# CrashCartCapital/rust-local-rag

Hardware: AMD Instinct MI355X
Metric: queries/sec, 768-d cosine top-100 over 10M chunks (single query, f32) (higher is better)
Workload: dtype f32

## Files before the change

### rust-local-rag_amd/csrc/exact.hip

```cpp
#include "common.h"
#include "exact_dot.h"
#include "staged_dot.h"
#include "sort_emit.h"
#include "kernels.h"
#include "../../include/rlr_gpu.h"

#include <algorithm>
#include <atomic>
#include <cstdlib>
#include <cstring>

namespace rlr {

namespace {

__device__ inline void stage_query(float *s_q, const float *__restrict__ query, uint32_t dim)
{
    for (uint32_t i = threadIdx.x; i < dim; i += blockDim.x)
        s_q[i] = query[i];
    __syncthreads();
}

template <bool F16>
__global__ __launch_bounds__(64) void rescore_kernel(const float4 *__restrict__ rows, uint32_t pitch16,
                                                     uint32_t dim, const float *__restrict__ query,
                                                     const uint32_t *__restrict__ cand,
                                                     const SelectState *__restrict__ st,
                                                     uint64_t *__restrict__ packed_out, uint32_t n_pad)
{
    extern __shared__ __attribute__((aligned(16))) float s_q[];
    stage_query(s_q, query, dim);
    const uint32_t n = min(st->n_cand, st->cap);
    const uint32_t i = blockIdx.x * 64 + threadIdx.x;
    if (i >= n_pad)
        return;
    if (i >= n) {
        packed_out[i] = 0;
        return;
    }
    const uint32_t r = cand[i];
    const float s = dot_ref_row<F16>(rows + static_cast<size_t>(r) * pitch16, s_q, dim);
    packed_out[i] = pack_result(s, r);
}

template <bool F16>
__global__ __launch_bounds__(256) void rescore_staged_kernel(const float4 *__restrict__ rows, uint32_t pitch16,
                                                             uint32_t dim, const float *__restrict__ query,
                                                             const uint32_t *__restrict__ cand,
                                                             const SelectState *__restrict__ st,
                                                             uint64_t *__restrict__ packed_out, uint32_t cpb,
                                                             uint32_t *__restrict__ hist_clear)
{
    extern __shared__ __attribute__((aligned(16))) float s_mem[];
    const uint32_t q_floats = (dim + 7) & ~7u;
    float *s_q = s_mem;
    float *s_p = s_mem + q_floats;
    const uint32_t tid = threadIdx.x;
    const uint32_t gid = blockIdx.x * 256 + tid;
    if (hist_clear && gid < 2 * kHistBins)
        hist_clear[gid] = 0;
    const uint32_t n = min(st->n_cand, st->cap);
    const uint32_t base = blockIdx.x * cpb;
    if (base >= n)
        return;
    const uint32_t cnt = min(cpb, n - base);
    __shared__ uint32_t s_cand[16];
    for (uint32_t i = tid; i < q_floats; i += 256)
        s_q[i] = i < dim ? query[i] : 0.0f;
    if (tid < cnt)
        s_cand[tid] = cand[base + tid];
    __syncthreads();
    const float sc = staged_reference_dot<F16>(rows, pitch16, dim, s_q, s_p, s_cand, cnt, tid);
    if (tid < cnt)
        packed_out[base + tid] = pack_result(sc, s_cand[tid]);
}

template <bool F16>
__global__ __launch_bounds__(256) void batch_rescore_kernel(const float4 *__restrict__ rows, uint32_t pitch16,
                                                            uint32_t dim, const float *__restrict__ queries,
                                                            uint32_t q_pitch, uint64_t *__restrict__ band,
                                                            uint32_t band_stride, const SelectState *__restrict__ st,
                                                            uint32_t cpb)
{
    extern __shared__ __attribute__((aligned(16))) float s_mem[];
    const uint32_t q_floats = (dim + 7) & ~7u;
    float *s_q = s_mem;
    float *s_p = s_mem + q_floats;
    __shared__ uint32_t s_cand[16];
    const uint32_t tid = threadIdx.x;
    const uint32_t q = blockIdx.y;
    const uint32_t n = st[q].pad;
    if (blockIdx.x * cpb >= n)
        return;
    const float *query = queries + static_cast<size_t>(q) * q_pitch;
    for (uint32_t i = tid; i < q_floats; i += 256)
        s_q[i] = i < dim ? query[i] : 0.0f;
    uint64_t *b = band + static_cast<size_t>(q) * band_stride;
    for (uint32_t base = blockIdx.x * cpb; base < n; base += gridDim.x * cpb) {
        const uint32_t cnt = min(cpb, n - base);
        __syncthreads();
        if (tid < cnt)
            s_cand[tid] = 0xFFFFFFFFu - static_cast<uint32_t>(b[base + tid] & 0xFFFFFFFFu);
        __syncthreads();
        const float sc = staged_reference_dot<F16>(rows, pitch16, dim, s_q, s_p, s_cand, cnt, tid);
        if (tid < cnt)
            b[base + tid] = pack_result(sc, s_cand[tid]);
    }
}

template <bool F16>
__global__ __launch_bounds__(64) void score_rows_kernel(const float4 *__restrict__ rows, uint32_t pitch16,
                                                        uint32_t dim, const float *__restrict__ query,
                                                        const uint32_t *__restrict__ list, uint32_t n,
                                                        float *__restrict__ out, const uint32_t *__restrict__ n_dev,
                                                        uint32_t n_rows_clamp)
{
    extern __shared__ __attribute__((aligned(16))) float s_q[];
    stage_query(s_q, query, dim);
    if (n_dev)
        n = min(n, *n_dev);
    const uint32_t i = blockIdx.x * 64 + threadIdx.x;
    if (i >= n)
        return;
    const uint32_t r = list[i] < n_rows_clamp ? list[i] : 0u;
    out[i] = dot_ref_row<F16>(rows + static_cast<size_t>(r) * pitch16, s_q, dim);
}

template <bool F16>
__global__ __launch_bounds__(64) void score_rows_batch_kernel(const float4 *__restrict__ rows, uint32_t pitch16, uint32_t dim,
                                                              const float *__restrict__ queries, uint32_t q_pitch,
                                                              const uint32_t *__restrict__ list, uint32_t stride,
                                                              float *__restrict__ out, const uint32_t *__restrict__ n_dev,
                                                              uint32_t n_dev_stride, uint32_t n_rows_clamp)
{
    const uint32_t q = blockIdx.y;
    const uint32_t n = min(stride, n_dev[static_cast<size_t>(q) * n_dev_stride]);
    if (blockIdx.x * 64 >= n)
        return;
    extern __shared__ __attribute__((aligned(16))) float s_q[];
    stage_query(s_q, queries + static_cast<size_t>(q) * q_pitch, dim);
    const uint32_t i = blockIdx.x * 64 + threadIdx.x;
    if (i >= n)
        return;
    const size_t at = static_cast<size_t>(q) * stride + i;
    const uint32_t r = list[at] < n_rows_clamp ? list[at] : 0u;
    out[at] = dot_ref_row<F16>(rows + static_cast<size_t>(r) * pitch16, s_q, dim);
}

template <bool F16>
__global__ __launch_bounds__(256) void score_rows_staged_kernel(const float4 *__restrict__ rows, uint32_t pitch16, uint32_t dim,
                                                               const float *__restrict__ query,
                                                               const uint32_t *__restrict__ list, uint32_t n,
                                                               float *__restrict__ out, uint32_t cpb,
                                                               const uint32_t *__restrict__ n_dev, uint32_t n_rows_clamp)
{
    extern __shared__ __attribute__((aligned(16))) float s_mem[];
    const uint32_t q_floats = (dim + 7) & ~7u;
    float *s_q = s_mem;
    float *s_p = s_mem + q_floats;
    __shared__ uint32_t s_cand[16];
    const uint32_t tid = threadIdx.x;
    const uint32_t base = blockIdx.x * cpb;
    if (n_dev)
        n = min(n, *n_dev);
    if (base >= n)
        return;
    const uint32_t cnt = min(cpb, n - base);
    for (uint32_t i = tid; i < q_floats; i += 256)
        s_q[i] = i < dim ? query[i] : 0.0f;
    if (tid < cnt) {
        const uint32_t r = list[base + tid];
        s_cand[tid] = r < n_rows_clamp ? r : 0u;
    }
    __syncthreads();
    const float sc = staged_reference_dot<F16>(rows, pitch16, dim, s_q, s_p, s_cand, cnt, tid);
    if (tid < cnt)
        out[base + tid] = sc;
}

__global__ __launch_bounds__(64) void sumsq_kernel(const float *__restrict__ staging, uint32_t n,
                                                   uint32_t dim, float *__restrict__ sumsq)
{
    const uint32_t r = blockIdx.x * 64 + threadIdx.x;
    if (r >= n)
        return;
    const float *v = staging + static_cast<size_t>(r) * dim;
    float s = 0.0f;
    for (uint32_t c = 0; c < dim; ++c) {
        float p = v[c] * v[c];
        s = s + p;
    }
    sumsq[r] = s;
}

__device__ inline float sqrt_rn(float x)
{
    float y = __builtin_sqrtf(x);
    const double xd = static_cast<double>(x);
#pragma unroll
    for (int it = 0; it < 2; ++it) {
        const uint32_t yb = __builtin_bit_cast(uint32_t, y);
        const float up = __builtin_bit_cast(float, yb + 1u);
        const float dn = __builtin_bit_cast(float, yb - 1u);
        const double m_hi = 0.5 * (static_cast<double>(y) + static_cast<double>(up));
        const double m_lo = 0.5 * (static_cast<double>(y) + static_cast<double>(dn));
        if (xd > m_hi * m_hi)
            y = up;
        else if (xd < m_lo * m_lo)
            y = dn;
    }
    return y;
}

__device__ inline float ref_scale(float v, float norm_sq, int do_normalize)
{
    if (do_normalize && norm_sq > 1e-20f)
        return __fdiv_rn(v, sqrt_rn(norm_sq));
    return v;
}

template <bool F16>
__global__ __launch_bounds__(256) void scale_store_kernel(const float *__restrict__ staging,
                                                          const float *__restrict__ sumsq, uint32_t n,
                                                          uint32_t dim, int do_normalize,
                                                          void *__restrict__ rows_out, uint32_t pitch16)
{
    const uint32_t pitch_e = F16 ? pitch16 * 8 : pitch16 * 4;
    const size_t total = static_cast<size_t>(n) * pitch_e;
    const size_t stride = static_cast<size_t>(gridDim.x) * 256;
    for (size_t i = static_cast<size_t>(blockIdx.x) * 256 + threadIdx.x; i < total; i += stride) {
        const uint32_t r = static_cast<uint32_t>(i / pitch_e);
        const uint32_t c = static_cast<uint32_t>(i - static_cast<size_t>(r) * pitch_e);
        float v = 0.0f;
        if (c < dim)
            v = ref_scale(staging[static_cast<size_t>(r) * dim + c], do_normalize ? sumsq[r] : 0.0f,
                          do_normalize);
        if constexpr (F16)
            static_cast<_Float16 *>(rows_out)[i] = static_cast<_Float16>(v);
        else
            static_cast<float *>(rows_out)[i] = v;
    }
}

__device__ inline uint64_t mix64(uint64_t z)
{
    z = (z ^ (z >> 30)) * 0xBF58476D1CE4E5B9ULL;
    z = (z ^ (z >> 27)) * 0x94D049BB133111EBULL;
    return z ^ (z >> 31);
}

__device__ inline int32_t ih4(uint64_t h)
{
    return static_cast<int32_t>((h & 0xFFFF) + ((h >> 16) & 0xFFFF) + ((h >> 32) & 0xFFFF) + (h >> 48)) - 131070;
}

__device__ inline float synth_raw(uint64_t s, uint64_t row, uint32_t col, uint32_t d, uint32_t n_clusters)
{
    const uint64_t idx = row * static_cast<uint64_t>(d) + col;
    int32_t t = ih4(mix64(s + (idx + 1) * 0x9E3779B97F4A7C15ULL));
    const bool tight = (n_clusters & 0x80000000u) != 0;
    n_clusters &= 0x7FFFFFFFu;
    if (n_clusters) {
        const uint64_t cl = mix64(s ^ (row + 0x632BE59BD9B4E019ULL)) % n_clusters;
        const uint64_t cidx = cl * static_cast<uint64_t>(d) + col;
        const int32_t c = ih4(mix64((s ^ 0xC1A57E55C1A57E55ULL) + (cidx + 1) * 0x9E3779B97F4A7C15ULL));
        if (tight)
            t = t / 16;
        t += 2 * c;
    }
    return static_cast<float>(t) * (1.0f / 65536.0f);
}

__global__ __launch_bounds__(64) void synth_sumsq_kernel(uint64_t s, uint64_t row0, uint32_t n, uint32_t dim,
                                                         uint32_t n_clusters, float *__restrict__ sumsq)
{
    const uint32_t r = blockIdx.x * 64 + threadIdx.x;
    if (r >= n)
        return;
    float acc = 0.0f;
    for (uint32_t c = 0; c < dim; ++c) {
        const float v = synth_raw(s, row0 + r, c, dim, n_clusters);
        float p = v * v;
        acc = acc + p;
    }
    sumsq[r] = acc;
}

template <bool F16>
__global__ __launch_bounds__(256) void synth_store_kernel(uint64_t s, uint64_t row0, uint32_t n, uint32_t dim,
                                                          uint32_t n_clusters, const float *__restrict__ sumsq,
                                                          void *__restrict__ rows_out, uint32_t pitch16)
{
    const uint32_t pitch_e = F16 ? pitch16 * 8 : pitch16 * 4;
    const size_t total = static_cast<size_t>(n) * pitch_e;
    const size_t stride = static_cast<size_t>(gridDim.x) * 256;
    for (size_t i = static_cast<size_t>(blockIdx.x) * 256 + threadIdx.x; i < total; i += stride) {
        const uint32_t r = static_cast<uint32_t>(i / pitch_e);
        const uint32_t c = static_cast<uint32_t>(i - static_cast<size_t>(r) * pitch_e);
        float v = 0.0f;
        if (c < dim)
            v = ref_scale(synth_raw(s, row0 + r, c, dim, n_clusters), sumsq[r], 1);
        if constexpr (F16)
            static_cast<_Float16 *>(rows_out)[i] = static_cast<_Float16>(v);
        else
            static_cast<float *>(rows_out)[i] = v;
    }
}

template <bool F16>
__global__ __launch_bounds__(256) void gather_f32_kernel(const void *__restrict__ rows, uint32_t pitch16,
                                                         uint32_t dim, const uint32_t *__restrict__ list,
                                                         uint32_t n, float *__restrict__ out)
{
    const size_t total = static_cast<size_t>(n) * dim;
    const size_t stride = static_cast<size_t>(gridDim.x) * 256;
    for (size_t i = static_cast<size_t>(blockIdx.x) * 256 + threadIdx.x; i < total; i += stride) {
        const uint32_t k = static_cast<uint32_t>(i / dim);
        const uint32_t c = static_cast<uint32_t>(i - static_cast<size_t>(k) * dim);
        const size_t r = list[k];
        if constexpr (F16)
            out[i] = h2f(static_cast<const uint16_t *>(rows)[r * pitch16 * 8 + c]);
        else
            out[i] = static_cast<const float *>(rows)[r * pitch16 * 4 + c];
    }
}

__global__ __launch_bounds__(256) void compact_rows_kernel(const float4 *__restrict__ src, float4 *__restrict__ dst,
                                                           uint32_t pitch16, const uint32_t *__restrict__ keep,
                                                           uint32_t n_keep)
{
    const size_t total = static_cast<size_t>(n_keep) * pitch16;
    const size_t stride = static_cast<size_t>(gridDim.x) * 256;
    for (size_t i = static_cast<size_t>(blockIdx.x) * 256 + threadIdx.x; i < total; i += stride) {
        const uint32_t k = static_cast<uint32_t>(i / pitch16);
        const uint32_t u = static_cast<uint32_t>(i - static_cast<size_t>(k) * pitch16);
        dst[i] = src[static_cast<size_t>(keep[k]) * pitch16 + u];
    }
}

__device__ inline bool finite_f(float x)
{
    return (__builtin_bit_cast(uint32_t, x) & 0x7F800000u) != 0x7F800000u;
}

__device__ inline float gram_entry(float dot)
{
    return finite_f(dot) ? dot : -__builtin_inff();
}

template <int SRC>
__device__ inline float4 gram_load4(const float *pool, const void *rows, uint32_t pitch16, uint32_t dim, uint32_t row, uint32_t col)
{
    if constexpr (SRC == 2) {
        const uint2 h = *reinterpret_cast<const uint2 *>(static_cast<const uint16_t *>(rows) + static_cast<size_t>(row) * pitch16 * 8 + col);
        return make_float4(h2f(static_cast<uint16_t>(h.x)), h2f(static_cast<uint16_t>(h.x >> 16)), h2f(static_cast<uint16_t>(h.y)),
                           h2f(static_cast<uint16_t>(h.y >> 16)));
    } else if constexpr (SRC == 1) {
        return *reinterpret_cast<const float4 *>(static_cast<const float *>(rows) + static_cast<size_t>(row) * pitch16 * 4 + col);
    } else {
        return *reinterpret_cast<const float4 *>(pool + static_cast<size_t>(row) * dim + col);
    }
}


template <int R, int SRC, int GK>
__global__ __launch_bounds__(256) void gram_tiled_kernel(const float *__restrict__ pool, uint32_t P, uint32_t dim,
                                                         float *__restrict__ gram, const void *__restrict__ rows,
                                                         uint32_t pitch16, const uint32_t *__restrict__ list)
{
    constexpr int kGT = 16 * R;
    constexpr int kGK = GK, kGPitch = GK + 4;
    __shared__ __attribute__((aligned(16))) float sa[kGT * kGPitch];
    __shared__ __attribute__((aligned(16))) float sb[kGT * kGPitch];
    if constexpr (SRC == 0)
        pool += static_cast<size_t>(blockIdx.z) * P * dim;
    else
        list += static_cast<size_t>(blockIdx.z) * P;
    gram += static_cast<size_t>(blockIdx.z) * P * P;
    uint32_t bi = 0, rem = blockIdx.x;
    while (rem > bi) {
        rem -= bi + 1;
        ++bi;
    }
    const uint32_t bj = rem;
    const uint32_t i0 = bi * kGT, j0 = bj * kGT;
    const uint32_t t = threadIdx.x, ty = t >> 4, tx = t & 15;
    float acc[R][R];
#pragma unroll
    for (int a = 0; a < R; ++a)
#pragma unroll
        for (int b = 0; b < R; ++b)
            acc[a][b] = 0.0f;
    const bool vec = (dim & 3u) == 0;
    constexpr int kPre = 2 * kGT * (kGK / 4) / 256;
    float4 pre[kPre];
    uint32_t src_row[kPre];
#pragma unroll
    for (int u = 0; u < kPre; ++u) {
        const uint32_t r = (t + 256 * u) / (kGK / 4);
        const uint32_t row = min(r >= kGT ? j0 + (r - kGT) : i0 + r, P - 1);
        src_row[u] = SRC == 0 ? row : list[row];
    }
    auto fetch = [&](uint32_t k0) {
        const uint32_t kc = min(static_cast<uint32_t>(kGK), dim - k0);
        if (vec) {
#pragma unroll
            for (int u = 0; u < kPre; ++u) {
                const uint32_t idx = t + 256 * u;
                const uint32_t r = idx / (kGK / 4), c4 = idx % (kGK / 4);
                const uint32_t row = r >= kGT ? j0 + (r - kGT) : i0 + r;
                const float4 v = gram_load4<SRC>(pool, rows, pitch16, dim, src_row[u], min(k0 + c4 * 4, dim - 4));
                pre[u] = (row < P && c4 * 4 < kc) ? v : make_float4(0.0f, 0.0f, 0.0f, 0.0f);
            }
            return;
        }
#pragma unroll
        for (int u = 0; u < kPre; ++u) {
            const uint32_t idx = t + 256 * u;
            const uint32_t r = idx / (kGK / 4), c4 = idx % (kGK / 4);
            const uint32_t row = r >= kGT ? j0 + (r - kGT) : i0 + r;
            float4 v = make_float4(0.0f, 0.0f, 0.0f, 0.0f);
            if (row < P && c4 * 4 < kc) {
                const uint32_t col = k0 + c4 * 4;
                if constexpr (SRC == 2) {
                    const uint16_t *src = static_cast<const uint16_t *>(rows) + static_cast<size_t>(src_row[u]) * pitch16 * 8 + col;
                    v.x = h2f(src[0]);
                    if (c4 * 4 + 1 < kc) v.y = h2f(src[1]);
                    if (c4 * 4 + 2 < kc) v.z = h2f(src[2]);
                    if (c4 * 4 + 3 < kc) v.w = h2f(src[3]);
                } else {
                    const float *src = SRC == 0 ? pool + static_cast<size_t>(row) * dim + col
                                                : static_cast<const float *>(rows) + static_cast<size_t>(src_row[u]) * pitch16 * 4 + col;
                    v.x = src[0];
                    if (c4 * 4 + 1 < kc) v.y = src[1];
                    if (c4 * 4 + 2 < kc) v.z = src[2];
                    if (c4 * 4 + 3 < kc) v.w = src[3];
                }
            }
            pre[u] = v;
        }
    };
    auto stash = [&]() {
#pragma unroll
        for (int u = 0; u < kPre; ++u) {
            const uint32_t idx = t + 256 * u;
            const uint32_t r = idx / (kGK / 4), c4 = idx % (kGK / 4);
            float *dst = (r >= kGT ? sb + (r - kGT) * kGPitch : sa + r * kGPitch) + c4 * 4;
            *reinterpret_cast<float4 *>(dst) = pre[u];
        }
    };
    fetch(0);
    stash();
    __syncthreads();
    for (uint32_t k0 = 0; k0 < dim; k0 += kGK) {
        const uint32_t kc = min(static_cast<uint32_t>(kGK), dim - k0);
        const bool more = k0 + kGK < dim;
        if (more)
            fetch(k0 + kGK);
        const uint32_t n4 = kc / 4;
        constexpr int kUnroll = R == 1 ? 8 : 1;
#pragma unroll kUnroll
        for (uint32_t c = 0; c < n4; ++c) {
            float4 xa[R], yb[R];
#pragma unroll
            for (int a = 0; a < R; ++a)
                xa[a] = reinterpret_cast<const float4 *>(sa + (ty + 16 * a) * kGPitch)[c];
#pragma unroll
            for (int b = 0; b < R; ++b)
                yb[b] = reinterpret_cast<const float4 *>(sb + (tx + 16 * b) * kGPitch)[c];
#pragma unroll
            for (int a = 0; a < R; ++a)
#pragma unroll
                for (int b = 0; b < R; ++b) {
                    float p;
                    p = xa[a].x * yb[b].x; acc[a][b] = acc[a][b] + p;
                    p = xa[a].y * yb[b].y; acc[a][b] = acc[a][b] + p;
                    p = xa[a].z * yb[b].z; acc[a][b] = acc[a][b] + p;
                    p = xa[a].w * yb[b].w; acc[a][b] = acc[a][b] + p;
                }
        }
        for (uint32_t e = n4 * 4; e < kc; ++e) {
#pragma unroll
            for (int a = 0; a < R; ++a)
#pragma unroll
                for (int b = 0; b < R; ++b) {
                    const float p = sa[(ty + 16 * a) * kGPitch + e] * sb[(tx + 16 * b) * kGPitch + e];
                    acc[a][b] = acc[a][b] + p;
                }
        }
        __syncthreads();
        if (more) {
            stash();
            __syncthreads();
        }
    }
#pragma unroll
    for (int a = 0; a < R; ++a)
#pragma unroll
        for (int b = 0; b < R; ++b) {
            const uint32_t ri = i0 + ty + 16 * a, cj = j0 + tx + 16 * b;
            if (ri < P && cj < P) {
                const float g = gram_entry(acc[a][b]);
                gram[static_cast<size_t>(ri) * P + cj] = g;
                gram[static_cast<size_t>(cj) * P + ri] = g;
            }
        }
}

__global__ __launch_bounds__(64) void mmr_greedy_kernel(const float *__restrict__ gram,
                                                        const float *__restrict__ scores, uint32_t P,
                                                        uint32_t k, float lambda, uint32_t *__restrict__ out_order,
                                                        float *__restrict__ out_mmr, uint32_t *__restrict__ out_n)
{
    extern __shared__ __attribute__((aligned(16))) unsigned char s_raw[];
    uint32_t *rem = reinterpret_cast<uint32_t *>(s_raw);
    float *max_sim = reinterpret_cast<float *>(s_raw) + P;
    float *rel = reinterpret_cast<float *>(s_raw) + 2 * P;
    const uint32_t lane = threadIdx.x;
    if (P == 0) {
        if (lane == 0)
            *out_n = 0;
        return;
    }
    for (uint32_t p = lane; p < P; p += 64) {
        rem[p] = p;
        max_sim[p] = 0.0f;
        rel[p] = scores[p];
    }
    __syncthreads();
    uint32_t n_rem = P, n_sel = 0;
    uint32_t last = rem[0];
    __syncthreads();
    if (lane == 0) {
        out_order[0] = last;
        out_mmr[0] = __builtin_bit_cast(float, 0x7FC00000u);
        rem[0] = rem[P - 1];
    }
    n_sel = 1;
    n_rem = P - 1;
    __syncthreads();

    const float one_minus = 1.0f - lambda;
    while (n_sel < k && n_rem > 0) {
        const float *g_last = gram + static_cast<size_t>(last) * P;
        uint64_t best = 0;
        for (uint32_t p = lane; p < n_rem; p += 64) {
            const uint32_t c = rem[p];
            const float sim = g_last[c];
            float ms = max_sim[c];
            if (finite_f(sim))
                ms = fmaxf(ms, sim);
            max_sim[c] = ms;
            const float r = rel[c];
            if (!finite_f(r))
                continue;
            const float t0 = one_minus * r;
            const float t1 = lambda * ms;
            float m = t0 - t1;
            if (!finite_f(m))
                continue;
            if (m == 0.0f)
                m = 0.0f;
            const uint64_t cand = (static_cast<uint64_t>(score_key(m)) << 32) | (0xFFFFFFFFu - p);
            if (cand > best)
                best = cand;
        }
#pragma unroll
        for (int off = 32; off > 0; off >>= 1) {
            const uint32_t hi = __shfl_xor(static_cast<uint32_t>(best >> 32), off);
            const uint32_t lo = __shfl_xor(static_cast<uint32_t>(best & 0xFFFFFFFFu), off);
            const uint64_t other = (static_cast<uint64_t>(hi) << 32) | lo;
            if (other > best)
                best = other;
        }
        if (best == 0)
            break;
        const uint32_t best_p = 0xFFFFFFFFu - static_cast<uint32_t>(best & 0xFFFFFFFFu);
        __syncthreads();
        last = rem[best_p];
        __syncthreads();
        if (lane == 0) {
            out_order[n_sel] = last;
            out_mmr[n_sel] = one_minus * rel[last] - lambda * max_sim[last];
            rem[best_p] = rem[n_rem - 1];
        }
        n_sel++;
        n_rem--;
        __syncthreads();
    }
    if (lane == 0)
        *out_n = n_sel;
}

template <typename Order>
__device__ __forceinline__ void emit_result_block(const MmrEmit &emit, uint32_t n_sel, uint32_t lane, Order order)
{
    const uint32_t status = emit.info[1];
    const uint32_t n = status ? 0u : min(n_sel, emit.k_cap);
    uint32_t chk = 0;
    for (uint32_t i = lane; i < n; i += 64) {
        const uint32_t o = order(i);
        const uint32_t w0 = emit.list[o], w1 = __builtin_bit_cast(uint32_t, emit.cosv[o]);
        const uint32_t w2 = __builtin_bit_cast(uint32_t, emit.comb[o]);
        const uint32_t w3 = emit.lexv ? __builtin_bit_cast(uint32_t, emit.lexv[o]) : 0u;
        emit.h_out[block_value(emit.k_cap, kBlockRow, i)] = w0;
        emit.h_out[block_value(emit.k_cap, kBlockCos, i)] = w1;
        emit.h_out[block_value(emit.k_cap, kBlockComb, i)] = w2;
        emit.h_out[block_value(emit.k_cap, kBlockLex, i)] = w3;
        chk += result_chk_term(w0, block_value(emit.k_cap, kBlockRow, i)) + result_chk_term(w1, block_value(emit.k_cap, kBlockCos, i)) +
               result_chk_term(w2, block_value(emit.k_cap, kBlockComb, i)) + result_chk_term(w3, block_value(emit.k_cap, kBlockLex, i));
    }
    __threadfence_system();
#pragma unroll
    for (int off = 32; off > 0; off >>= 1)
        chk += static_cast<uint32_t>(__shfl_xor(static_cast<int>(chk), off));
    if (lane == 0) {
        emit.h_out[block_n(emit.k_cap)] = n;
        emit.h_out[block_status(emit.k_cap)] = status;
        emit.h_out[block_chk(emit.k_cap)] = block_chk_tail(chk, n, status, emit.k_cap);
        __threadfence_system();
        emit.h_out[block_done(emit.k_cap)] = kBlockDone;
    }
}

__device__ __forceinline__ void emit_empty_block(const MmrEmit &emit)
{
    const uint32_t status = emit.info[1];
    emit.h_out[block_n(emit.k_cap)] = 0;
    emit.h_out[block_status(emit.k_cap)] = status;
    emit.h_out[block_chk(emit.k_cap)] = block_chk_tail(0u, 0u, status, emit.k_cap);
    __threadfence_system();
    emit.h_out[block_done(emit.k_cap)] = kBlockDone;
}

template <int J>
__device__ inline float lane_max_skip_nan(const float (&v)[J])
{
    float best = -__builtin_inff();
    int j = 0;
#pragma unroll
    for (; j + 1 < J; j += 2)
        asm("v_max3_f32 %0, %1, %2, %3" : "=v"(best) : "v"(best), "v"(v[j]), "v"(v[j + 1]));
    if (j < J)
        asm("v_max_f32 %0, %1, %2" : "=v"(best) : "v"(best), "v"(v[j]));
    return best;
}

template <int J>
__global__ __launch_bounds__(256) void mmr_greedy_lazy_kernel(const float *__restrict__ gram, const float *__restrict__ scores,
                                                              uint32_t P, uint32_t k, float lambda,
                                                              uint32_t *__restrict__ out_order, float *__restrict__ out_mmr,
                                                              uint32_t *__restrict__ out_n, const uint32_t *__restrict__ sizes,
                                                              MmrEmit emit)
{
    constexpr uint32_t kSlots = 64 * J;
    __shared__ uint2 s_log[kSlots];
    __shared__ uint16_t s_rem[kSlots], s_posof[kSlots];
    {
        const uint32_t stride = P;
        gram += static_cast<size_t>(blockIdx.x) * stride * stride;
        scores += static_cast<size_t>(blockIdx.x) * stride;
        out_order += static_cast<size_t>(blockIdx.x) * stride;
        out_mmr += static_cast<size_t>(blockIdx.x) * stride;
        out_n += blockIdx.x;
    }
    const uint32_t g_stride = P;
    if (sizes)
        P = sizes[blockIdx.x];
    if (P == 0) {
        if (threadIdx.x == 0) {
            *out_n = 0;
            if (emit.h_out)
                emit_empty_block(emit);
        }
        return;
    }
    {
        const float4 *g4 = reinterpret_cast<const float4 *>(gram);
        const uint32_t n4 = (P * g_stride) / 4;
        float warm = 0.0f;
        for (uint32_t i = threadIdx.x * 8; i < n4; i += 256 * 8)
            warm += g4[i].x;
        asm volatile("" ::"v"(warm));
    }
    __syncthreads();
    if (threadIdx.x >= 64)
        return;
    const uint32_t lane = threadIdx.x;
    for (uint32_t c = lane; c < P; c += 64) {
        s_rem[c] = static_cast<uint16_t>(c);
        s_posof[c] = static_cast<uint16_t>(c);
    }
    float t0[J], ms[J];
    uint32_t idx[J];
    const float one_minus = 1.0f - lambda;
    const float nan_f = __builtin_bit_cast(float, 0x7FC00000u);
    const float neg_inf = -__builtin_inff();
#pragma unroll
    for (int j = 0; j < J; ++j) {
        const uint32_t c = lane + 64 * j;
        idx[j] = min(c, P - 1);
        const float t = one_minus * scores[idx[j]];
        t0[j] = ((c < P) & (c != 0) & finite_f(t)) ? t : nan_f;
        ms[j] = 0.0f;
    }
    uint32_t n_sel = 1, last = 0, replayed = 0;
    s_log[0] = make_uint2(0u, 0x7FC00000u);
    while (n_sel < k && n_sel < P) {
        const float *g_last = gram + static_cast<size_t>(last) * g_stride;
        float sim[J];
#pragma unroll
        for (int j = 0; j < J; ++j)
            sim[j] = g_last[idx[j]];
        float m0[J];
#pragma unroll
        for (int j = 0; j < J; ++j) {
            ms[j] = sim[j] > ms[j] ? sim[j] : ms[j];
            const float t1 = lambda * ms[j];
            m0[j] = t0[j] - t1;
        }
        float wm = wave_max_f32_no_nan(lane_max_skip_nan<J>(m0));
        if (wm == __builtin_inff()) {
#pragma unroll
            for (int j = 0; j < J; ++j)
                m0[j] = finite_f(m0[j]) ? m0[j] : nan_f;
            wm = wave_max_f32_no_nan(lane_max_skip_nan<J>(m0));
        }
        if (wm == neg_inf)
            break;
        auto take = [&](const bool (&hit)[J]) {
            uint32_t win = 0;
#pragma unroll
            for (int j = 0; j < J; ++j) {
                win = hit[j] ? lane + 64 * j + 1 : win;
                t0[j] = hit[j] ? nan_f : t0[j];
            }
            const int src = __builtin_ctzll(__ballot(win != 0));
            last = static_cast<uint32_t>(__builtin_amdgcn_readlane(static_cast<int>(win), src)) - 1;
            float wm_raw = wm;
            if (wm == 0.0f) {
                float z = 0.0f;
#pragma unroll
                for (int j = 0; j < J; ++j)
                    z = hit[j] ? m0[j] : z;
                wm_raw = __builtin_bit_cast(float, __builtin_amdgcn_readlane(__builtin_bit_cast(int, z), src));
            }
            s_log[n_sel] = make_uint2(last, __builtin_bit_cast(uint32_t, wm_raw));
            __builtin_amdgcn_fence(__ATOMIC_RELEASE, "wavefront");
            __builtin_amdgcn_wave_barrier();
            n_sel++;
        };
        bool hit[J];
        uint32_t holders = 0;
#pragma unroll
        for (int j = 0; j < J; ++j) {
            hit[j] = m0[j] == wm;
            holders += static_cast<uint32_t>(__builtin_popcountll(__ballot(hit[j])));
        }
        if (holders == 1) {
            take(hit);
            continue;
        }
        if (lane == 0) {
            for (uint32_t i = replayed; i < n_sel; ++i) {
                const uint32_t w = s_log[i].x, n = P - i;
                const uint32_t p = s_posof[w], moved = s_rem[n - 1];
                s_rem[p] = static_cast<uint16_t>(moved);
                s_posof[moved] = static_cast<uint16_t>(p);
            }
        }
        __builtin_amdgcn_fence(__ATOMIC_RELEASE, "wavefront");
        __builtin_amdgcn_wave_barrier();
        __builtin_amdgcn_fence(__ATOMIC_ACQUIRE, "wavefront");
        replayed = n_sel;
        uint32_t pj[J], bp = 0xFFFFFFFFu;
#pragma unroll
        for (int j = 0; j < J; ++j) {
            pj[j] = hit[j] ? static_cast<uint32_t>(s_posof[idx[j]]) : 0xFFFFFFFFu;
            bp = min(bp, pj[j]);
        }
        const uint32_t wp = wave_min_u32(bp);
        bool first[J];
#pragma unroll
        for (int j = 0; j < J; ++j)
            first[j] = pj[j] == wp;
        take(first);
    }
    for (uint32_t i = lane; i < n_sel; i += 64) {
        const uint2 e = s_log[i];
        out_order[i] = e.x;
        out_mmr[i] = __builtin_bit_cast(float, e.y);
    }
    if (lane == 0)
        *out_n = n_sel;
    if (emit.h_out)
        emit_result_block(emit, n_sel, lane, [&](uint32_t i) { return s_log[i].x; });
}

uint32_t ew_blocks(size_t total)
{
    size_t b = (total + 255) / 256;
    if (b > 256 * 16) b = 256 * 16;
    return b ? static_cast<uint32_t>(b) : 1u;
}

}

hipError_t launch_rescore(const void *rows, uint32_t pitch16, uint32_t dim, int dtype, const float *query,
                          const uint32_t *cand, const SelectState *st, uint64_t *packed_out, uint32_t n_pad,
                          hipStream_t s)
{
    const uint32_t blocks = (n_pad + 63) / 64;
    const size_t lds = static_cast<size_t>(dim) * sizeof(float);
    const float4 *r4 = static_cast<const float4 *>(rows);
    if (dtype == RLR_F16)
        hipLaunchKernelGGL(rescore_kernel<true>, dim3(blocks), dim3(64), lds, s, r4, pitch16, dim, query, cand, st,
                           packed_out, n_pad);
    else
        hipLaunchKernelGGL(rescore_kernel<false>, dim3(blocks), dim3(64), lds, s, r4, pitch16, dim, query, cand, st,
                           packed_out, n_pad);
    return hipGetLastError();
}

bool launch_rescore_staged(const void *rows, uint32_t pitch16, uint32_t dim, int dtype, const float *query,
                           const uint32_t *cand, const SelectState *st, uint64_t *packed_out, uint32_t n_max,
                           uint32_t *hist_clear, hipStream_t s, hipError_t *err)
{
    const size_t q_bytes = static_cast<size_t>((dim + 7) & ~7u) * sizeof(float);
    const size_t row_bytes = q_bytes + 16;
    if (pitch16 * (dtype == RLR_F16 ? 8u : 4u) < ((dim + 7) & ~7u))
        return false;
    uint32_t cpb = 8;
    while (cpb > 1 && q_bytes + cpb * row_bytes > 60 * 1024)
        cpb >>= 1;
    if (q_bytes + cpb * row_bytes > 60 * 1024)
        return false;
    const uint32_t blocks = std::max<uint32_t>((n_max + cpb - 1) / cpb, (2 * kHistBins + 255) / 256);
    const size_t lds = q_bytes + cpb * row_bytes;
    const float4 *r4 = static_cast<const float4 *>(rows);
    if (dtype == RLR_F16)
        hipLaunchKernelGGL(rescore_staged_kernel<true>, dim3(blocks), dim3(256), lds, s, r4, pitch16, dim, query, cand,
                           st, packed_out, cpb, hist_clear);
    else
        hipLaunchKernelGGL(rescore_staged_kernel<false>, dim3(blocks), dim3(256), lds, s, r4, pitch16, dim, query, cand,
                           st, packed_out, cpb, hist_clear);
    *err = hipGetLastError();
    return true;
}

bool batch_rescore_fits(uint32_t pitch16, uint32_t dim, int dtype)
{
    const size_t q_bytes = static_cast<size_t>((dim + 7) & ~7u) * sizeof(float);
    if (pitch16 * (dtype == RLR_F16 ? 8u : 4u) < ((dim + 7) & ~7u))
        return false;
    return 2 * q_bytes + 16 <= 60 * 1024;
}

bool launch_batch_rescore(const void *rows, uint32_t pitch16, uint32_t dim, int dtype, const float *queries,
                          uint32_t q_pitch, uint32_t n_queries, uint64_t *band, uint32_t band_stride,
                          const SelectState *st, hipStream_t s, hipError_t *err)
{
    const size_t q_bytes = static_cast<size_t>((dim + 7) & ~7u) * sizeof(float);
    const size_t row_bytes = q_bytes + 16;
    if (pitch16 * (dtype == RLR_F16 ? 8u : 4u) < ((dim + 7) & ~7u))
        return false;
    uint32_t cpb = 8;
    while (cpb > 1 && q_bytes + cpb * row_bytes > 60 * 1024)
        cpb >>= 1;
    if (q_bytes + cpb * row_bytes > 60 * 1024)
        return false;
    const size_t lds = q_bytes + cpb * row_bytes;
    const float4 *r4 = static_cast<const float4 *>(rows);
    const dim3 grid(32, n_queries);
    if (dtype == RLR_F16)
        hipLaunchKernelGGL(batch_rescore_kernel<true>, grid, dim3(256), lds, s, r4, pitch16, dim, queries, q_pitch, band,
                           band_stride, st, cpb);
    else
        hipLaunchKernelGGL(batch_rescore_kernel<false>, grid, dim3(256), lds, s, r4, pitch16, dim, queries, q_pitch, band,
                           band_stride, st, cpb);
    *err = hipGetLastError();
    return true;
}

hipError_t launch_score_rows(const void *rows, uint32_t pitch16, uint32_t dim, int dtype, const float *query,
                             const uint32_t *list, uint32_t n, float *cos_out, hipStream_t s, const uint32_t *n_dev,
                             uint32_t n_rows_clamp)
{
    if (n == 0)
        return hipSuccess;
    const float4 *r4 = static_cast<const float4 *>(rows);
    const size_t q_bytes = static_cast<size_t>((dim + 7) & ~7u) * sizeof(float);
    const size_t row_bytes = q_bytes + 16;
    uint32_t cpb = 8;
    while (cpb > 1 && q_bytes + cpb * row_bytes > 60 * 1024)
        cpb >>= 1;
    const bool fits = q_bytes + cpb * row_bytes <= 60 * 1024 && pitch16 * (dtype == RLR_F16 ? 8u : 4u) >= ((dim + 7) & ~7u);
    if (fits && n > 64) {
        const uint32_t blocks = (n + cpb - 1) / cpb;
        const size_t lds = q_bytes + cpb * row_bytes;
        if (dtype == RLR_F16)
            hipLaunchKernelGGL(score_rows_staged_kernel<true>, dim3(blocks), dim3(256), lds, s, r4, pitch16, dim, query, list, n,
                               cos_out, cpb, n_dev, n_rows_clamp);
        else
            hipLaunchKernelGGL(score_rows_staged_kernel<false>, dim3(blocks), dim3(256), lds, s, r4, pitch16, dim, query, list, n,
                               cos_out, cpb, n_dev, n_rows_clamp);
        return hipGetLastError();
    }
    const uint32_t blocks = (n + 63) / 64;
    const size_t lds = static_cast<size_t>(dim) * sizeof(float);
    if (dtype == RLR_F16)
        hipLaunchKernelGGL(score_rows_kernel<true>, dim3(blocks), dim3(64), lds, s, r4, pitch16, dim, query, list, n,
                           cos_out, n_dev, n_rows_clamp);
    else
        hipLaunchKernelGGL(score_rows_kernel<false>, dim3(blocks), dim3(64), lds, s, r4, pitch16, dim, query, list, n,
                           cos_out, n_dev, n_rows_clamp);
    return hipGetLastError();
}

hipError_t launch_score_rows_batch(const void *rows, uint32_t pitch16, uint32_t dim, int dtype, const float *queries,
                                   uint32_t q_pitch, uint32_t n_queries, const uint32_t *list, uint32_t stride, float *cos_out,
                                   const uint32_t *n_dev, uint32_t n_dev_stride, uint32_t n_rows_clamp, hipStream_t s)
{
    if (stride == 0 || n_queries == 0)
        return hipSuccess;
    const float4 *r4 = static_cast<const float4 *>(rows);
    const dim3 grid((stride + 63) / 64, n_queries);
    const size_t lds = static_cast<size_t>(dim) * sizeof(float);
    if (dtype == RLR_F16)
        hipLaunchKernelGGL(score_rows_batch_kernel<true>, grid, dim3(64), lds, s, r4, pitch16, dim, queries, q_pitch, list, stride,
                           cos_out, n_dev, n_dev_stride, n_rows_clamp);
    else
        hipLaunchKernelGGL(score_rows_batch_kernel<false>, grid, dim3(64), lds, s, r4, pitch16, dim, queries, q_pitch, list, stride,
                           cos_out, n_dev, n_dev_stride, n_rows_clamp);
    return hipGetLastError();
}

hipError_t launch_normalize_store(float *staging, uint32_t n, uint32_t dim, int do_normalize, void *rows_out,
                                  uint32_t pitch16, int dtype, float *norm_tmp, hipStream_t s)
{
    if (n == 0)
        return hipSuccess;
    hipLaunchKernelGGL(sumsq_kernel, dim3((n + 63) / 64), dim3(64), 0, s, staging, n, dim, norm_tmp);
    const size_t total = static_cast<size_t>(n) * pitch16 * (dtype == RLR_F16 ? 8 : 4);
    if (dtype == RLR_F16)
        hipLaunchKernelGGL(scale_store_kernel<true>, dim3(ew_blocks(total)), dim3(256), 0, s, staging, norm_tmp, n,
                           dim, do_normalize, rows_out, pitch16);
    else
        hipLaunchKernelGGL(scale_store_kernel<false>, dim3(ew_blocks(total)), dim3(256), 0, s, staging, norm_tmp, n,
                           dim, do_normalize, rows_out, pitch16);
    return hipGetLastError();
}

hipError_t launch_synth(void *rows_out, uint32_t pitch16, uint32_t dim, int dtype, uint64_t row0, uint32_t n,
                        uint64_t seed, uint32_t n_clusters, float *norm_tmp, hipStream_t s)
{
    if (n == 0)
        return hipSuccess;
    uint64_t z = seed ^ 0x5EED5EED5EED5EEDULL;
    z = (z ^ (z >> 30)) * 0xBF58476D1CE4E5B9ULL;
    z = (z ^ (z >> 27)) * 0x94D049BB133111EBULL;
    z = z ^ (z >> 31);
    hipLaunchKernelGGL(synth_sumsq_kernel, dim3((n + 63) / 64), dim3(64), 0, s, z, row0, n, dim, n_clusters,
                       norm_tmp);
    const size_t total = static_cast<size_t>(n) * pitch16 * (dtype == RLR_F16 ? 8 : 4);
    if (dtype == RLR_F16)
        hipLaunchKernelGGL(synth_store_kernel<true>, dim3(ew_blocks(total)), dim3(256), 0, s, z, row0, n, dim,
                           n_clusters, norm_tmp, rows_out, pitch16);
    else
        hipLaunchKernelGGL(synth_store_kernel<false>, dim3(ew_blocks(total)), dim3(256), 0, s, z, row0, n, dim,
                           n_clusters, norm_tmp, rows_out, pitch16);
    return hipGetLastError();
}

hipError_t launch_gather_f32(const void *rows, uint32_t pitch16, uint32_t dim, int dtype, const uint32_t *list,
                             uint32_t n, float *out, hipStream_t s)
{
    if (n == 0)
        return hipSuccess;
    const size_t total = static_cast<size_t>(n) * dim;
    if (dtype == RLR_F16)
        hipLaunchKernelGGL(gather_f32_kernel<true>, dim3(ew_blocks(total)), dim3(256), 0, s, rows, pitch16, dim, list,
                           n, out);
    else
        hipLaunchKernelGGL(gather_f32_kernel<false>, dim3(ew_blocks(total)), dim3(256), 0, s, rows, pitch16, dim,
                           list, n, out);
    return hipGetLastError();
}

hipError_t launch_compact_rows(const void *src, void *dst, uint32_t pitch16, const uint32_t *keep, uint32_t n_keep,
                               hipStream_t s)
{
    if (n_keep == 0)
        return hipSuccess;
    const size_t total = static_cast<size_t>(n_keep) * pitch16;
    hipLaunchKernelGGL(compact_rows_kernel, dim3(ew_blocks(total)), dim3(256), 0, s,
                       static_cast<const float4 *>(src), static_cast<float4 *>(dst), pitch16, keep, n_keep);
    return hipGetLastError();
}

typedef float v32f __attribute__((ext_vector_type(32)));

__global__ __launch_bounds__(64) void gram_mfma_f32_kernel(const unsigned char *__restrict__ rows, uint32_t pitch_bytes,
                                                           uint32_t dim, const uint32_t *__restrict__ list, uint32_t P,
                                                           uint32_t n_pools, uint32_t jobs_per_pool, float *__restrict__ gram)
{
    constexpr int UPR = 4;
    constexpr int kGmPitch = UPR * 16 + 16;
    constexpr int kPer = 96 * UPR / 64;
    __shared__ __attribute__((aligned(16))) unsigned char s_rows[96 * kGmPitch];
    const uint32_t xcd = blockIdx.x & 7u, slot = blockIdx.x >> 3;
    const uint32_t pool = (slot / jobs_per_pool) * 8 + xcd;
    if (pool >= n_pools)
        return;
    const uint32_t nb = (P + 31) / 32;
    uint32_t p = 0, rem = slot % jobs_per_pool;
    while (rem >= nb - 2 * p) {
        rem -= nb - 2 * p;
        ++p;
    }
    const uint32_t I0 = 2 * p, J = 2 * p + rem;
    list += static_cast<size_t>(pool) * P;
    gram += static_cast<size_t>(pool) * P * P;
    const uint32_t lane = threadIdx.x;
    const unsigned char *src[kPer];
#pragma unroll
    for (int i = 0; i < kPer; ++i) {
        const uint32_t u = lane + 64 * i, rr = u / UPR, seg = u % UPR;
        const uint32_t row = min(rr < 64 ? I0 * 32 + rr : J * 32 + (rr - 64), P - 1);
        src[i] = rows + static_cast<size_t>(list[row]) * pitch_bytes + seg * 16;
    }
    const uint32_t seg = lane % UPR;
    const uint32_t row_units = pitch_bytes / 16;
    const uint32_t n_chunks = (row_units + UPR - 1) / UPR;
    const uint32_t tail_unit = dim / 8, tail_keep = dim % 8;
    const auto half_mask = [&](uint32_t j) { return tail_keep >= 2 * j + 2 ? 0xFFFFFFFFu : tail_keep == 2 * j + 1 ? 0xFFFFu : 0u; };
    const uint4 tail_mask = make_uint4(half_mask(0), half_mask(1), half_mask(2), half_mask(3));
    uint4 pre[kPer];
    auto fetch = [&](uint32_t c) {
        const bool in = c * UPR + seg < row_units;
#pragma unroll
        for (int i = 0; i < kPer; ++i)
            pre[i] = in ? *reinterpret_cast<const uint4 *>(src[i] + static_cast<size_t>(c) * (UPR * 16)) : make_uint4(0u, 0u, 0u, 0u);
        if (tail_keep && c * UPR + seg == tail_unit) {
#pragma unroll
            for (int i = 0; i < kPer; ++i)
                pre[i] = make_uint4(pre[i].x & tail_mask.x, pre[i].y & tail_mask.y, pre[i].z & tail_mask.z, pre[i].w & tail_mask.w);
        }
    };
    v32f acc;
#pragma unroll
    for (int i = 0; i < 32; ++i)
        acc[i] = 0.0f;
    const unsigned char *la = s_rows + lane * kGmPitch;
    const unsigned char *lb = s_rows + (64 + (lane & 31)) * kGmPitch;
    fetch(0);
    for (uint32_t c = 0; c < n_chunks; ++c) {
#pragma unroll
        for (int i = 0; i < kPer; ++i)
            *reinterpret_cast<uint4 *>(s_rows + ((lane + 64 * i) / UPR) * kGmPitch + seg * 16) = pre[i];
        __builtin_amdgcn_fence(__ATOMIC_RELEASE, "wavefront");
        if (c + 1 < n_chunks)
            fetch(c + 1);
#pragma unroll
        for (int u = 0; u < UPR; ++u) {
            const uint4 ca = *reinterpret_cast<const uint4 *>(la + u * 16), cb = *reinterpret_cast<const uint4 *>(lb + u * 16);
            const uint32_t wa[4] = {ca.x, ca.y, ca.z, ca.w}, wb[4] = {cb.x, cb.y, cb.z, cb.w};
#pragma unroll
            for (int j = 0; j < 4; ++j) {
                acc = __builtin_amdgcn_mfma_f32_32x32x1f32(h2f(static_cast<uint16_t>(wa[j] & 0xFFFF)), h2f(static_cast<uint16_t>(wb[j] & 0xFFFF)), acc, 0, 0, 0);
                acc = __builtin_amdgcn_mfma_f32_32x32x1f32(h2f(static_cast<uint16_t>(wa[j] >> 16)), h2f(static_cast<uint16_t>(wb[j] >> 16)), acc, 0, 0, 0);
            }
        }
        __builtin_amdgcn_fence(__ATOMIC_ACQUIRE, "wavefront");
    }
    const uint32_t jcol = J * 32 + (lane & 31);
#pragma unroll
    for (int v = 0; v < 32; ++v) {
        const uint32_t i = (I0 + v / 16) * 32 + 8 * ((v % 16) / 4) + 4 * (lane >> 5) + (v % 4);
        if (i < P && jcol < P) {
            const float g = gram_entry(acc[v]);
            gram[static_cast<size_t>(i) * P + jcol] = g;
            gram[static_cast<size_t>(jcol) * P + i] = g;
        }
    }
}

template <int SRC>
static hipError_t launch_gram_src(const float *pool, uint32_t P, uint32_t dim, float *gram, uint32_t n_queries,
                                  const void *rows, uint32_t pitch16, const uint32_t *list, hipStream_t s)
{
    if (n_queries >= 8) {
        const uint32_t nb = (P + 63) / 64;
        hipLaunchKernelGGL((gram_tiled_kernel<4, SRC, 64>), dim3(nb * (nb + 1) / 2, 1, n_queries), dim3(256), 0, s, pool, P, dim,
                           gram, rows, pitch16, list);
    } else {
        const uint32_t nb1 = (P + 15) / 16;
        if (static_cast<uint64_t>(nb1) * (nb1 + 1) / 2 * n_queries <= 512) {
            hipLaunchKernelGGL((gram_tiled_kernel<1, SRC, 384>), dim3(nb1 * (nb1 + 1) / 2, 1, n_queries), dim3(256), 0, s, pool, P,
                               dim, gram, rows, pitch16, list);
        } else if (static_cast<uint64_t>(nb1) * (nb1 + 1) / 2 * n_queries <= 1536) {
            hipLaunchKernelGGL((gram_tiled_kernel<1, SRC, 128>), dim3(nb1 * (nb1 + 1) / 2, 1, n_queries), dim3(256), 0, s, pool, P,
                               dim, gram, rows, pitch16, list);
        } else {
            const uint32_t nb = (P + 31) / 32;
            hipLaunchKernelGGL((gram_tiled_kernel<2, SRC, 64>), dim3(nb * (nb + 1) / 2, 1, n_queries), dim3(256), 0, s, pool, P, dim,
                               gram, rows, pitch16, list);
        }
    }
    return hipGetLastError();
}

hipError_t launch_gram(const float *pool, uint32_t P, uint32_t dim, float *gram, uint32_t n_queries, hipStream_t s)
{
    if (P == 0 || n_queries == 0)
        return hipSuccess;
    return launch_gram_src<0>(pool, P, dim, gram, n_queries, nullptr, 0, nullptr, s);
}

hipError_t launch_gram_rows(const void *rows, uint32_t pitch16, uint32_t dim, int dtype, const uint32_t *list, uint32_t P,
                            float *gram, uint32_t n_queries, hipStream_t s)
{
    if (P == 0 || n_queries == 0)
        return hipSuccess;
    if (dtype == RLR_F16) {
        if (n_queries >= 16) {
            const uint32_t nb = (P + 31) / 32;
            uint32_t jobs_per_pool = 0;
            for (uint32_t pr = 0; 2 * pr < nb; ++pr)
                jobs_per_pool += nb - 2 * pr;
            const uint32_t pools8 = (n_queries + 7) / 8 * 8;
            hipLaunchKernelGGL(gram_mfma_f32_kernel, dim3(pools8 * jobs_per_pool), dim3(64), 0, s, static_cast<const unsigned char *>(rows),
                               pitch16 * 16u, dim, list, P, n_queries, jobs_per_pool, gram);
            return hipGetLastError();
        }
        return launch_gram_src<2>(nullptr, P, dim, gram, n_queries, rows, pitch16, list, s);
    }
    return launch_gram_src<1>(nullptr, P, dim, gram, n_queries, rows, pitch16, list, s);
}

hipError_t launch_mmr_greedy(const float *gram, const float *scores, uint32_t P, uint32_t k, float lambda,
                             uint32_t *out_order, float *out_mmr, uint32_t *out_n, const uint32_t *sizes,
                             uint32_t n_queries, hipStream_t s, const MmrEmit *emit_in)
{
    const size_t lds = static_cast<size_t>(P ? P : 1) * 12;
    const MmrEmit emit = emit_in ? *emit_in : MmrEmit{};
    if (emit.h_out && (n_queries != 1 || P == 0 || P > 1024))
        return hipErrorInvalidValue;
#define RLR_MMR_REG(JV)                                                                                          \
    hipLaunchKernelGGL(mmr_greedy_lazy_kernel<JV>, dim3(n_queries), dim3(256), 0, s, gram, scores, P, k, lambda, \
                       out_order, out_mmr, out_n, sizes, emit)
    if (P == 0 || (P > 1024 && n_queries == 1 && !sizes))
        hipLaunchKernelGGL(mmr_greedy_kernel, dim3(1), dim3(64), lds, s, gram, scores, P, k, lambda, out_order, out_mmr,
                           out_n);
    else if (P > 1024)
        return hipErrorInvalidValue;
    else if (P <= 64)
        RLR_MMR_REG(1);
    else if (P <= 128)
        RLR_MMR_REG(2);
    else if (P <= 320)
        RLR_MMR_REG(5);
    else if (P <= 512)
        RLR_MMR_REG(8);
    else
        RLR_MMR_REG(16);
#undef RLR_MMR_REG
    return hipGetLastError();
}

}
```

Measured before the change: 225.1.

## Add fast-path MMR greedy loop with DPP wave max and early row prefetch

Restructures the MMR greedy selection loop so the common case (a single finite, non-zero winner held by one lane) runs in a tight inner loop. That loop uses a hand-written DPP wave-max reduction ending in a scalar readlane, and a packed tag summed across J slots to pick the winner with one ballot and one readlane. The next gram row is fetched right after the winner is known, with byte offsets precomputed, so the load overlaps the bookkeeping that follows. Ties, infinities, zero and NaN cases fall back to the original slow path, which now also issues the row fetch; this adds inline-asm complexity and carries a risk of DPP hazard or correctness mistakes.

```diff
diff --git a/rust-local-rag_amd/csrc/exact.hip b/rust-local-rag_amd/csrc/exact.hip
--- a/rust-local-rag_amd/csrc/exact.hip
+++ b/rust-local-rag_amd/csrc/exact.hip
@@ -647,6 +647,38 @@
 }
 
 template <int J>
+__device__ inline float wave_max_skip_nan(const float (&v)[J])
+{
+    float best = -__builtin_inff();
+    int j = 0;
+#pragma unroll
+    for (; j + 4 < J; j += 2)
+        asm("v_max3_f32 %0, %1, %2, %3" : "=v"(best) : "v"(best), "v"(v[j]), "v"(v[j + 1]));
+#define RLR_WAVE_MAX_TAIL                                                          \
+    "s_nop 1\n\tv_max_f32_dpp %1, %1, %1 row_shr:1 row_mask:0xf bank_mask:0xf\n\t"   \
+    "s_nop 1\n\tv_max_f32_dpp %1, %1, %1 row_shr:2 row_mask:0xf bank_mask:0xf\n\t"   \
+    "s_nop 1\n\tv_max_f32_dpp %1, %1, %1 row_shr:4 row_mask:0xf bank_mask:0xf\n\t"   \
+    "s_nop 1\n\tv_max_f32_dpp %1, %1, %1 row_shr:8 row_mask:0xf bank_mask:0xf\n\t"   \
+    "s_nop 1\n\tv_max_f32_dpp %1, %1, %1 row_bcast:15 row_mask:0xa bank_mask:0xf\n\t" \
+    "s_nop 1\n\tv_max_f32_dpp %1, %1, %1 row_bcast:31 row_mask:0xc bank_mask:0xf\n\t" \
+    "s_nop 1\n\tv_readlane_b32 %0, %1, 63"
+    float wm;
+    if constexpr (J % 2 == 0) {
+        if constexpr (J >= 4) {
+            asm("v_max3_f32 %0, %1, %2, %3" : "=v"(best) : "v"(best), "v"(v[J - 4]), "v"(v[J - 3]));
+        }
+        asm volatile("v_max3_f32 %1, %1, %2, %3\n\t" RLR_WAVE_MAX_TAIL : "=s"(wm), "+v"(best) : "v"(v[J - 2]), "v"(v[J - 1]));
+    } else if constexpr (J >= 3) {
+        asm("v_max3_f32 %0, %1, %2, %3" : "=v"(best) : "v"(best), "v"(v[J - 3]), "v"(v[J - 2]));
+        asm volatile("v_max_f32 %1, %1, %2\n\t" RLR_WAVE_MAX_TAIL : "=s"(wm), "+v"(best) : "v"(v[J - 1]));
+    } else {
+        asm volatile("v_max_f32 %1, %1, %2\n\t" RLR_WAVE_MAX_TAIL : "=s"(wm), "+v"(best) : "v"(v[J - 1]));
+    }
+#undef RLR_WAVE_MAX_TAIL
+    return wm;
+}
+
+template <int J>
 __global__ __launch_bounds__(256) void mmr_greedy_lazy_kernel(const float *__restrict__ gram, const float *__restrict__ scores,
                                                               uint32_t P, uint32_t k, float lambda,
                                                               uint32_t *__restrict__ out_order, float *__restrict__ out_mmr,
@@ -693,6 +725,9 @@
     }
     float t0[J], ms[J];
     uint32_t idx[J];
+    uint32_t off[J];
+    uint32_t tag[J];
+    constexpr uint32_t kOne = 0x10000u;
     const float one_minus = 1.0f - lambda;
     const float nan_f = __builtin_bit_cast(float, 0x7FC00000u);
     const float neg_inf = -__builtin_inff();
@@ -703,23 +738,64 @@
         const float t = one_minus * scores[idx[j]];
         t0[j] = ((c < P) & (c != 0) & finite_f(t)) ? t : nan_f;
         ms[j] = 0.0f;
+        off[j] = idx[j] * 4u;
+        tag[j] = kOne + c;
+        asm volatile("" : "+v"(off[j]), "+v"(tag[j]));
     }
     uint32_t n_sel = 1, last = 0, replayed = 0;
     s_log[0] = make_uint2(0u, 0x7FC00000u);
-    while (n_sel < k && n_sel < P) {
-        const float *g_last = gram + static_cast<size_t>(last) * g_stride;
-        float sim[J];
-#pragma unroll
-        for (int j = 0; j < J; ++j)
-            sim[j] = g_last[idx[j]];
-        float m0[J];
+    float sim[J];
+    auto fetch_row = [&]() {
+        const char *g_last = reinterpret_cast<const char *>(gram) + last * g_stride * 4u;
 #pragma unroll
         for (int j = 0; j < J; ++j) {
-            ms[j] = sim[j] > ms[j] ? sim[j] : ms[j];
-            const float t1 = lambda * ms[j];
-            m0[j] = t0[j] - t1;
-        }
-        float wm = wave_max_f32_no_nan(lane_max_skip_nan<J>(m0));
+            asm volatile("" : "+v"(off[j]));
+            sim[j] = *reinterpret_cast<const float *>(g_last + off[j]);
+        }
+    };
+    fetch_row();
+    const uint32_t n_max = min(k, P);
+    float m0[J], wm = 0.0f;
+    for (;;) {
+        if (n_sel >= n_max)
+            break;
+        bool go;
+        do {
+            go = false;
+#pragma unroll
+            for (int j = J - 1; j >= 0; --j) {
+                asm("v_max_f32 %0, %1, %2" : "=v"(ms[j]) : "v"(ms[j]), "v"(sim[j]));
+                const float t1 = lambda * ms[j];
+                m0[j] = t0[j] - t1;
+            }
+            wm = wave_max_skip_nan<J>(m0);
+            const uint32_t wm2 = __builtin_bit_cast(uint32_t, wm) << 1;
+            if (__builtin_expect(wm2 - 1u < 0xFEFFFFFFu, 1)) {
+                uint32_t held = 0;
+#pragma unroll
+                for (int j = 0; j < J; ++j)
+                    held += m0[j] == wm ? tag[j] : 0u;
+                const uint64_t lanes = __ballot(held != 0);
+                const int src = __builtin_ctzll(lanes);
+                uint32_t s = 2 * kOne;
+                if (__builtin_expect(lanes == 1ull << src, 1))
+                    s = static_cast<uint32_t>(__builtin_amdgcn_readlane(static_cast<int>(held), src));
+                if (__builtin_expect(s < 2 * kOne, 1)) {
+                    last = s - kOne;
+                    fetch_row();
+#pragma unroll
+                    for (int j = 0; j < J; ++j)
+                        t0[j] = m0[j] == wm ? nan_f : t0[j];
+                    s_log[n_sel] = make_uint2(last, __builtin_bit_cast(uint32_t, wm));
+                    __builtin_amdgcn_fence(__ATOMIC_RELEASE, "wavefront");
+                    __builtin_amdgcn_wave_barrier();
+                    n_sel++;
+                    go = n_sel < n_max;
+                }
+            }
+        } while (go);
+        if (n_sel >= n_max)
+            break;
         if (wm == __builtin_inff()) {
 #pragma unroll
             for (int j = 0; j < J; ++j)
@@ -737,6 +813,7 @@
             }
             const int src = __builtin_ctzll(__ballot(win != 0));
             last = static_cast<uint32_t>(__builtin_amdgcn_readlane(static_cast<int>(win), src)) - 1;
+            fetch_row();
             float wm_raw = wm;
             if (wm == 0.0f) {
                 float z = 0.0f;
```

After: 220.6. 0.98x the previous value.
